# himhan34/Intensity_based_LiDAR_SLAM_for_me-

Measured on AMD Instinct MI355X. Metric: scans/sec (64×1024 Ouster) feature+kNN+residual path; pose Δ vs CPU ref, higher is better.
Workload: dtype fp32 features / fp64 residual+solve

## Files before the change

include/lislam.h:

```cpp
#ifndef LISLAM_H_
#define LISLAM_H_

#include <stddef.h>
#include <stdint.h>

#ifdef __cplusplus
extern "C" {
#endif

#define LISLAM_OK 0
#define LISLAM_ERR_ARG (-1)
#define LISLAM_ERR_DEVICE (-2)
#define LISLAM_ERR_CAPACITY (-3)
#define LISLAM_ERR_STATE (-4)

typedef struct lislam_ctx lislam_ctx;
typedef struct lislam_batch lislam_batch;
typedef struct lislam_odom lislam_odom;

typedef struct {
  int32_t n_scans;
  int32_t width;
  float min_range;
  int32_t max_iterations;
// ... 57 lines not shown
#define LISLAM_OUT_LASER_CLOUD 3
#define LISLAM_OUT_CURVATURE 4
#define LISLAM_OUT_LABEL 5
#define LISLAM_OUT_LINE_OFFSETS 6
#define LISLAM_OUT_SHARP 7
#define LISLAM_OUT_LESS_SHARP 8
#define LISLAM_OUT_FLAT 9
#define LISLAM_OUT_LESS_FLAT 10
#define LISLAM_OUT_PARA 11
#define LISLAM_OUT_POSE 12
#define LISLAM_OUT_STATS 13
#define LISLAM_OUT_ORB_T 14
#define LISLAM_OUT_ORB_STATS 15
#define LISLAM_OUT_ORB_KEYPOINTS 16
#define LISLAM_OUT_ORB_POINTS 17
#define LISLAM_OUT_ORB_DESCRIPTORS 18
#define LISLAM_OUT_GROUND 19
#define LISLAM_OUT_GROUND_PLANE 20
#define LISLAM_OUT_GROUND_INFO 21
int lislam_batch_download(lislam_batch* b, int32_t what, int32_t scan, void* dst, int32_t cap, int32_t* n);
int lislam_batch_download_cloud(lislam_batch* b, int32_t what, int32_t scan, void* dst, const lislam_point_layout* layout,
                                int32_t cap, int32_t* n);

#define LISLAM_ENGINE_OFF 0
#define LISLAM_ENGINE_AUTO 1
#define LISLAM_ENGINE_ON 2
int lislam_set_odometry_schedule(lislam_ctx* ctx, int32_t mode);
int lislam_set_engine_shape(lislam_ctx* ctx, int32_t queries_per_wave, int32_t depth);
#define LISLAM_PAIRING_OFF 0
#define LISLAM_PAIRING_AUTO 1
#define LISLAM_PAIRING_REQUIRE 2
int lislam_set_engine_pairing(lislam_ctx* ctx, int32_t mode);
int lislam_batch_odometry_paired(lislam_batch* b, int32_t* paired);
int lislam_batch_odometry_status(lislam_batch* b, int32_t* status);
int lislam_batch_odometry_engine(lislam_batch* b, int32_t* kind);
int lislam_batch_odometry_abort_code(lislam_batch* b, int32_t* code);
int lislam_device_queue_count(int32_t device, int32_t* masked_queues);

#define LISLAM_TIES_REFERENCE 0
#define LISLAM_TIES_INDEX 1
int lislam_set_tie_order(lislam_ctx* ctx, int32_t order);

int lislam_eval_factors(lislam_ctx* ctx, int32_t n, const int32_t* kind, const double* pts, const double* q,
                        const double* t, double* residuals, double* jac);
int lislam_eval_factors_raw(lislam_ctx* ctx, int32_t n, const int32_t* kind, const double* pts, const double* q,
                            const double* t, double* residuals, double* jac_q, double* jac_t);
// ... 145 lines not shown
```

intensity_based_lidar_slam_for_me-_amd/csrc/lislam_abi.cpp:

```cpp
#include <hip/hip_runtime.h>

#include <algorithm>
#include <atomic>
#include <cstdarg>
#include <cstdio>
#include <cstdlib>
#include <cstring>
#include <string>
#include <vector>

#include "../../include/lislam.h"
#include "lislam_batch.hpp"
#include "lislam_ctx.hpp"
#include "lislam_internal.hpp"

using namespace lislam;


namespace {

int fail(lislam_ctx* c, int code, const char* fmt, ...) {
  if (c) {
    char buf[512];
    va_list ap;
// ... 655 lines not shown
}

int lislam_batch_odometry_engine(lislam_batch* b, int32_t* kind) {
  if (!b || !kind) return LISLAM_ERR_ARG;
  *kind = !b->engine_ran ? 0 : b->eng_split == 1 ? 2 : 1;
  return LISLAM_OK;
}

int lislam_batch_kernel_times(lislam_batch* b, float* ms_per_call, int32_t* launches_per_call, int32_t* calls) {
  if (!b || !ms_per_call) return LISLAM_ERR_ARG;
  SETTLE(b);
  lislam_ctx* c = b->ctx;
  hipSetDevice(c->device);
  HIPCHK(c, hipStreamSynchronize(c->stream));
  double acc[LISLAM_NUM_KERNELS] = {0};
  int launches[LISLAM_NUM_KERNELS] = {0};
  auto el = [&](hipEvent_t a0, hipEvent_t a1) -> double {
    float ms = 0;
    if (hipEventElapsedTime(&ms, a0, a1) != hipSuccess) return 0.0;
    return ms;
  };
  for (auto& v : b->ext_ev) {
    timeline_print(c->device, "extract", b, 0, v[0], v[4]);
    for (int i = 0; i < 4; i++) { acc[i] += el(v[i], v[i + 1]); launches[i] += i == 3 ? 2 : i == 0 ? 3 : 1; }
    for (hipEvent_t e : v) b->pool.push_back(e);
  }
  for (auto& v : b->odo_ev) {
    for (auto& t : v) {
      timeline_print(c->device, "odometry", b, t.kernel, t.b, t.e);
      acc[t.kernel] += el(t.b, t.e);
      launches[t.kernel] += 1;
      b->pool.push_back(t.b);
      b->pool.push_back(t.e);
    }
  }
  const int ne = (int)b->ext_ev.size(), no = (int)b->odo_ev.size();
  for (int k = 0; k < LISLAM_NUM_KERNELS; k++) {
    const int ncall = k < 4 ? ne : no;
    ms_per_call[k] = ncall ? (float)(acc[k] / ncall) : 0.f;
    if (launches_per_call) launches_per_call[k] = ncall ? launches[k] / ncall : 0;
  }
  if (calls) { calls[0] = ne; calls[1] = no; }
  b->ext_ev.clear();
  b->odo_ev.clear();
  return LISLAM_OK;
}

// ... 151 lines not shown
  if (info && (rc = lislam_batch_download(b, LISLAM_OUT_GROUND_INFO, 0, info, 4, &n))) return rc;
  if (out) {
    if ((rc = lislam_batch_download(b, LISLAM_OUT_GROUND, 0, out, cap, &n))) return rc;
    if (n_out) *n_out = n;
  }
  return LISLAM_OK;
}

int lislam_odom_create(lislam_ctx* c, lislam_odom** out) {
  if (!c || !out) return LISLAM_ERR_ARG;
  hipSetDevice(c->device);
  int rc = ensure_single(c);
  if (rc) return rc;
  *out = new lislam_odom();
  (*out)->ctx = c;
  return LISLAM_OK;
}

int lislam_odom_destroy(lislam_odom* od) {
  delete od;
  return LISLAM_OK;
}

static int put_frame(lislam_batch* b, int slot, const lislam_frame* fr) {
  lislam_ctx* c = b->ctx;
  if (fr->n_sharp > b->cap_sharp || fr->n_less_sharp > b->cap_less_sharp || fr->n_flat > b->cap_flat ||
      fr->n_less_flat > b->N || fr->n_sharp < 0 || fr->n_less_sharp < 0 || fr->n_flat < 0 || fr->n_less_flat < 0)
    return fail(c, LISLAM_ERR_CAPACITY, "frame exceeds feature capacities");
  const FeatureArgs& f = b->fa;
  auto cp = [&](P4* dst, const float* src, int n) -> int {
    if (n > 0) HIPCHK(c, hipMemcpyAsync(dst, src, (size_t)n * 16, hipMemcpyHostToDevice, c->stream));
    return LISLAM_OK;
  };
  int rc = 0;
  rc |= cp(f.sharp + (size_t)slot * b->cap_sharp, fr->sharp, fr->n_sharp);
  rc |= cp(f.less_sharp + (size_t)slot * b->cap_less_sharp, fr->less_sharp, fr->n_less_sharp);
  rc |= cp(f.flat + (size_t)slot * b->cap_flat, fr->flat, fr->n_flat);
  rc |= cp(f.less_flat + (size_t)slot * b->N, fr->less_flat, fr->n_less_flat);
  const int cnt[4] = {fr->n_sharp, fr->n_less_sharp, fr->n_flat, fr->n_less_flat};
  HIPCHK(c, hipMemcpyAsync(f.n_feat + slot * 4, cnt, sizeof(cnt), hipMemcpyHostToDevice, c->stream));
  const int H = b->H;
  std::vector<int> loff(2 * (H + 1));
  const float* src[2] = {fr->less_sharp, fr->less_flat};
  const int nsrc[2] = {fr->n_less_sharp, fr->n_less_flat};
  for (int w = 0; w < 2; w++) {
    int j = 0;
    for (int l = 0; l <= H; l++) {
      while (j < nsrc[w] && (l == H || (int)src[w][4 * j + 3] < l)) j++;
      loff[w * (H + 1) + l] = j;
    }
  }
  HIPCHK(c, hipMemcpyAsync(f.feat_loff + (size_t)slot * 2 * (H + 1), loff.data(), loff.size() * sizeof(int),
                           hipMemcpyHostToDevice, c->stream));
  OdomArgs o = b->oa;
  o.less_sharp = f.less_sharp + (size_t)slot * b->cap_less_sharp;
  o.less_flat = f.less_flat + (size_t)slot * b->N;
  o.sharp = f.sharp + (size_t)slot * b->cap_sharp;
  o.flat = f.flat + (size_t)slot * b->cap_flat;
  o.qpts_sharp += (size_t)slot * b->cap_sharp;
  o.qpts_flat += (size_t)slot * b->cap_flat;
  o.n_feat = f.n_feat + slot * 4;
  for (TargetIndex* ti : {&o.idx_ls, &o.idx_lf}) {
    ti->chunk += (size_t)slot * ti->nchunk * 2;
    ti->super += (size_t)slot * ti->nsuper * 2;
    ti->nn_chunk += (size_t)slot * ti->nchunk * 2;
    ti->nn_super += (size_t)slot * ti->nsuper * 2;
    ti->sorted += (size_t)slot * ti->cap;
    ti->keys += (size_t)slot * 2 * ti->cap;
  }
  launch_target_index(o, 1, c->stream);
  HIPCHK(c, hipGetLastError());
  HIPCHK(c, hipStreamSynchronize(c->stream));
  return rc ? LISLAM_ERR_DEVICE : LISLAM_OK;
}

static int copy_slot(lislam_batch* b, int from, int to) {
  lislam_ctx* c = b->ctx;
  const hipStream_t st = c->stream;
  auto cp = [&](const void* base, size_t per_slot) -> int {
    const char* p = static_cast<const char*>(base);
    HIPCHK(c, hipMemcpyAsync(const_cast<char*>(p) + (size_t)to * per_slot, p + (size_t)from * per_slot, per_slot,
                             hipMemcpyDeviceToDevice, st));
    return LISLAM_OK;
  };
  const FeatureArgs& f = b->fa;
  const OdomArgs& o = b->oa;
  int rc = 0;
  rc |= cp(f.sharp, (size_t)b->cap_sharp * 16);
  rc |= cp(f.less_sharp, (size_t)b->cap_less_sharp * 16);
  rc |= cp(f.flat, (size_t)b->cap_flat * 16);
  rc |= cp(f.less_flat, (size_t)b->N * 16);
  rc |= cp(f.n_feat, 4 * sizeof(int));
  rc |= cp(f.feat_loff, (size_t)2 * (b->H + 1) * sizeof(int));
  for (const TargetIndex* ti : {&o.idx_ls, &o.idx_lf}) {
// ... 165 lines not shown
```

intensity_based_lidar_slam_for_me-_amd/csrc/lislam_internal.hpp:

```cpp
#pragma once
#include <hip/hip_runtime.h>
#include <stdint.h>

#include <atomic>
#include <chrono>
#include <vector>

#include "lislam_device.hpp"

namespace lislam {

constexpr int kMaxLines = 128;
constexpr int kCapSharpPerLine = 12;
constexpr int kCapLessSharpPerLine = 120;
constexpr int kCapFlatPerLine = 24;
constexpr int kMaxEngineDepth = 6;

struct FeatureArgs {
  const P4* pts;
  int S, H, W, N;
  float min_range;
  uint8_t* img_range;
  uint8_t* img_int;
  P4* track;
// ... 61 lines not shown
  const int* gate;
  unsigned* eng_ctl;
  int eng_qpw, eng_depth;
  int* warm;
  double* eng_part;
};

struct FactorArgs {
  int n;
  const int* kind;
  const double* pts;
  const double* x;
  double* res;
  double* jac;
};

struct WireLayout {
  uint32_t step, ox, oy, oz, oi;
};
void launch_unpack_layout(const uint8_t* raw, int n, const WireLayout& L, P4* out, hipStream_t st);
void launch_pack_layout(const P4* in, int n, const WireLayout& L, uint8_t* raw, hipStream_t st);

void launch_features(const FeatureArgs& a, hipStream_t st, hipEvent_t* ev , hipEvent_t images_ready);
void launch_target_index(const OdomArgs& a, int n_scans, hipStream_t st);
struct OdoTimed {
  int kernel;
  hipEvent_t b, e;
};
void launch_odometry(const OdomArgs& a, const hipStream_t* streams, int ngroups, hipEvent_t fork,
                     const hipEvent_t* join, std::vector<OdoTimed>* ev, hipEvent_t (*get_event)(void*),
                     void* ev_owner);
int launch_odometry_chain(const OdomArgs& a, hipStream_t st);
int launch_odometry_chain_split(const OdomArgs& a, hipEvent_t ready, hipEvent_t fork, hipEvent_t join_r,
                                hipEvent_t join_i, hipEvent_t t0, hipEvent_t t1, unsigned* h_abort, hipEvent_t done);
struct EngineRequest {
  OdomArgs a;
  hipEvent_t ready, fork, join_r, join_i, t0, t1, done;
  unsigned* h_abort;
  void* plan = nullptr;
  std::atomic<int> state{0};
  int pairing = 0;
  size_t ctl_words = 0;
  bool paired = false;
  bool held = false;
  std::chrono::steady_clock::time_point hold_t0;
};
// ... 28 lines not shown
```

intensity_based_lidar_slam_for_me-_amd/csrc/lislam_odometry.hip:

```cpp
#include <hip/hip_runtime.h>
#include <hip/hip_ext.h>

#include <algorithm>
#include <atomic>
#include <cassert>
#include <chrono>
#include <condition_variable>
#include <cstdlib>
#include <cstring>
#include <deque>
#include <mutex>
#include <thread>
#include <vector>

#include "lislam_device.hpp"
#include "lislam_factors.hpp"
#include "lislam_internal.hpp"
#include "lislam_lm.hpp"
#include "lislam_lm_wave.hpp"

namespace lislam {

__device__ __forceinline__ int uni(int v) { return __builtin_amdgcn_readfirstlane(v); }

constexpr double kDistSq = 25.0;
constexpr double kNearby = 2.5;


__device__ __forceinline__ uint32_t spread10(uint32_t v) {
  v &= 0x3ffu;
  v = (v | (v << 16)) & 0x030000FFu;
  v = (v | (v << 8)) & 0x0300F00Fu;
  v = (v | (v << 4)) & 0x030C30C3u;
  v = (v | (v << 2)) & 0x09249249u;
  return v;
}

__device__ __forceinline__ void stg4(float4* p, float4 v) {
  f4v w = {v.x, v.y, v.z, v.w};
  *(gf4v_mut*)p = w;
}

__device__ __forceinline__ void chunk_boxes(const float4* pts, int n, bool label_from_w, float4* chunk, float4* super) {
  const int nch = (n + kChunk - 1) / kChunk;
  for (int c = threadIdx.x; c < nch; c += blockDim.x) {
    float4 lo = make_float4(3.4e38f, 3.4e38f, 3.4e38f, 1e9f), hi = make_float4(-3.4e38f, -3.4e38f, -3.4e38f, -1e9f);
    for (int j = c * kChunk; j < min(n, c * kChunk + kChunk); j++) {
      const float4 p = ldg(pts + j);
      const float l = label_from_w ? (float)int(p.w) : 0.f;
      lo.x = fminf(lo.x, p.x); lo.y = fminf(lo.y, p.y); lo.z = fminf(lo.z, p.z); lo.w = fminf(lo.w, l);
      hi.x = fmaxf(hi.x, p.x); hi.y = fmaxf(hi.y, p.y); hi.z = fmaxf(hi.z, p.z); hi.w = fmaxf(hi.w, l);
    }
    stg4(chunk + 2 * c, lo);
    stg4(chunk + 2 * c + 1, hi);
  }
  __syncthreads();
  const int nsu = (nch + kChunk - 1) / kChunk;
  for (int c = threadIdx.x; c < nsu; c += blockDim.x) {
    float4 lo = make_float4(3.4e38f, 3.4e38f, 3.4e38f, 1e9f), hi = make_float4(-3.4e38f, -3.4e38f, -3.4e38f, -1e9f);
    for (int k = c * kChunk; k < min(nch, c * kChunk + kChunk); k++) {
      const float4 l = ldg(chunk + 2 * k), h = ldg(chunk + 2 * k + 1);
      lo.x = fminf(lo.x, l.x); lo.y = fminf(lo.y, l.y); lo.z = fminf(lo.z, l.z); lo.w = fminf(lo.w, l.w);
      hi.x = fmaxf(hi.x, h.x); hi.y = fmaxf(hi.y, h.y); hi.z = fmaxf(hi.z, h.z); hi.w = fmaxf(hi.w, h.w);
    }
    stg4(super + 2 * c, lo);
    stg4(super + 2 * c + 1, hi);
  }
  __syncthreads();
}

typedef __attribute__((address_space(1))) uint64_t gu64;

__device__ __forceinline__ void global_bitonic(gu64* keys, int P) {
  for (int k = 2; k <= P; k <<= 1) {
    for (int j = k >> 1; j > 0; j >>= 1) {
      for (int i = threadIdx.x; i < P; i += blockDim.x) {
        const int ixj = i ^ j;
        if (ixj > i) {
          const uint64_t x = keys[i], y = keys[ixj];
          if ((x > y) == ((i & k) == 0)) { keys[i] = y; keys[ixj] = x; }
        }
      }
      __syncthreads();
    }
  }
}

template <int kW, int kK>
__device__ __forceinline__ void wg_bitonic(uint64_t (&key)[kK], int P, uint64_t* xch) {
  constexpr int kPer = 64 * kK;
  const int w = threadIdx.x >> 6, lane = lane_id();
  const bool active = w * kPer < P;
  const int base = w * kPer;
  for (int k = 2; k <= P; k <<= 1) {
    for (int j = k >> 1; j >= kPer; j >>= 1) {
      const int pw = w ^ (j / kPer);
      const bool up = (base & k) == 0, lower = (w & (j / kPer)) == 0;
#pragma unroll
      for (int h = 0; h < kK / 8; h++) {
        if (active)
#pragma unroll
          for (int t = 0; t < 8; t++) xch[(w * 8 + t) * 64 + lane] = key[h * 8 + t];
        __syncthreads();
        if (active)
#pragma unroll
          for (int t = 0; t < 8; t++) {
            const uint64_t x = key[h * 8 + t], y = xch[(pw * 8 + t) * 64 + lane];
            key[h * 8 + t] = (lower == up) ? (x < y ? x : y) : (x < y ? y : x);
          }
        __syncthreads();
      }
    }
    if (active) reg_bitonic_level<kK>(key, k, min(k >> 1, kPer / 2), base);
  }
}

#ifndef LISLAM_TI_WPE32
#define LISLAM_TI_WPE32 4
#endif
template <int kW, int kK>
__device__ __forceinline__ void target_index_body(const OdomArgs& a, int bid, int per_scan, int w0, int w1, int w2,
                                                  uint64_t* xch, float (*red)[kW]) {
  constexpr int kKeysPerLane = kK, kPer = 64 * kK;
  const int s = bid / per_scan, wi = bid % per_scan;
  const int which = wi == 0 ? w0 : wi == 1 ? w1 : w2;
  const bool query = which >= 2;
  const TargetIndex& ix = (which & 1) ? a.idx_lf : a.idx_ls;
  const float4* pts = reinterpret_cast<const float4*>(
      which == 0 ? a.less_sharp + (size_t)s * a.cap_less_sharp : which == 1 ? a.less_flat + (size_t)s * a.N
      : which == 2 ? a.sharp + (size_t)s * a.cap_sharp : a.flat + (size_t)s * a.cap_flat);
  const int n = a.n_feat[s * 4 + (which == 0 ? 1 : which == 1 ? 3 : which == 2 ? 0 : 2)];
  if (!query) chunk_boxes(pts, n, true, ix.chunk + (size_t)s * ix.nchunk * 2, ix.super + (size_t)s * ix.nsuper * 2);
  if (n == 0) return;
  float mn[3] = {3.4e38f, 3.4e38f, 3.4e38f}, mx[3] = {-3.4e38f, -3.4e38f, -3.4e38f};
  if (!query) {
    const float4* sb = ix.super + (size_t)s * ix.nsuper * 2;
    const int nsu = ((n + kChunk - 1) / kChunk + kChunk - 1) / kChunk;
    for (int u = threadIdx.x; u < nsu; u += 64 * kW) {
      const float4 l = ldg(sb + 2 * u), h = ldg(sb + 2 * u + 1);
      mn[0] = fminf(mn[0], l.x); mn[1] = fminf(mn[1], l.y); mn[2] = fminf(mn[2], l.z);
      mx[0] = fmaxf(mx[0], h.x); mx[1] = fmaxf(mx[1], h.y); mx[2] = fmaxf(mx[2], h.z);
    }
  } else {
    for (int j = threadIdx.x; j < n; j += 64 * kW) {
      const float4 p = ldg(pts + j);
      mn[0] = fminf(mn[0], p.x); mn[1] = fminf(mn[1], p.y); mn[2] = fminf(mn[2], p.z);
      mx[0] = fmaxf(mx[0], p.x); mx[1] = fmaxf(mx[1], p.y); mx[2] = fmaxf(mx[2], p.z);
    }
  }
  for (int d = 0; d < 3; d++)
    for (int o = 32; o > 0; o >>= 1) {
      mn[d] = fminf(mn[d], __shfl_xor(mn[d], o));
      mx[d] = fmaxf(mx[d], __shfl_xor(mx[d], o));
    }
  const int lane = threadIdx.x & 63, wave = threadIdx.x >> 6;
// ... 35 lines not shown
      for (int t = 0; t < kKeysPerLane; t++) {
        const int i = wave * kPer + t * 64 + lane;
        if (i < n) f(i, (int)(uint32_t)key[t]);
      }
    } else {
      for (int i = threadIdx.x; i < n; i += 64 * kW) f(i, (int)(uint32_t)gkeys[i]);
    }
  };
  if (query) {
    float4* qp = which == 2 ? a.qpts_sharp + (size_t)s * a.cap_sharp : a.qpts_flat + (size_t)s * a.cap_flat;
    emit([&](int i, int o) {
      const float4 p = ldg(pts + o);
      stg4(qp + i, make_float4(p.x, p.y, p.z, __int_as_float(o)));
    });
    return;
  }
  float4* sorted = ix.sorted + (size_t)s * ix.cap;
  if (!in_regs) {
    emit([&](int i, int o) {
      const float4 p = ldg(pts + o);
      stg4(sorted + i, make_float4(p.x, p.y, p.z, __int_as_float(o)));
    });
    __syncthreads();
    chunk_boxes(sorted, n, false, ix.nn_chunk + (size_t)s * ix.nchunk * 2, ix.nn_super + (size_t)s * ix.nsuper * 2);
    return;
  }
  float4* nch_out = ix.nn_chunk + (size_t)s * ix.nchunk * 2;
  float4* nsu_out = ix.nn_super + (size_t)s * ix.nsuper * 2;
  auto rmin = [](float v) {
    v = fminf(v, __int_as_float(__builtin_amdgcn_mov_dpp(__float_as_int(v), 0xB1, 0xf, 0xf, true)));
    v = fminf(v, __int_as_float(__builtin_amdgcn_mov_dpp(__float_as_int(v), 0x4E, 0xf, 0xf, true)));
    v = fminf(v, __int_as_float(__builtin_amdgcn_mov_dpp(__float_as_int(v), 0x141, 0xf, 0xf, true)));
    return fminf(v, __int_as_float(__builtin_amdgcn_mov_dpp(__float_as_int(v), 0x140, 0xf, 0xf, true)));
  };
  float slo[3] = {3.4e38f, 3.4e38f, 3.4e38f}, shi[3] = {-3.4e38f, -3.4e38f, -3.4e38f};
#pragma unroll
  for (int t = 0; t < kKeysPerLane; t++) {
    const int i = wave * kPer + t * 64 + lane;
    float4 p = make_float4(3.4e38f, 3.4e38f, 3.4e38f, 0.f);
    float q[3] = {-3.4e38f, -3.4e38f, -3.4e38f};
    if (i < n) {
      const int o = (int)(uint32_t)key[t];
      p = ldg(pts + o);
      stg4(sorted + i, make_float4(p.x, p.y, p.z, __int_as_float(o)));
      q[0] = p.x; q[1] = p.y; q[2] = p.z;
    }
    const float lo0 = rmin(p.x), lo1 = rmin(p.y), lo2 = rmin(p.z);
    const float hi0 = -rmin(-q[0]), hi1 = -rmin(-q[1]), hi2 = -rmin(-q[2]);
    const int c = i >> 4;
    if ((lane & 15) == 0 && i < n) {
      stg4(nch_out + 2 * c, make_float4(lo0, lo1, lo2, 0.f));
      stg4(nch_out + 2 * c + 1, make_float4(hi0, hi1, hi2, 0.f));
    }
    slo[0] = fminf(slo[0], lo0); slo[1] = fminf(slo[1], lo1); slo[2] = fminf(slo[2], lo2);
    shi[0] = fmaxf(shi[0], hi0); shi[1] = fmaxf(shi[1], hi1); shi[2] = fmaxf(shi[2], hi2);
    if ((t & 3) == 3) {
      float r[6] = {slo[0], slo[1], slo[2], -shi[0], -shi[1], -shi[2]};
#pragma unroll
      for (int e = 0; e < 6; e++) {
        float v = r[e];
        v = fminf(v, __int_as_float(__builtin_amdgcn_ds_swizzle(__float_as_int(v), (16 << 10) | 0x1f)));
        v = fminf(v, __shfl_xor(v, 32));
        r[e] = v;
      }
      const int u = (wave * kPer + (t - 3) * 64) >> 8;
      if (lane == 0 && u * kSuper < n) {
        stg4(nsu_out + 2 * u, make_float4(r[0], r[1], r[2], 0.f));
        stg4(nsu_out + 2 * u + 1, make_float4(-r[3], -r[4], -r[5], 0.f));
      }
      slo[0] = slo[1] = slo[2] = 3.4e38f;
      shi[0] = shi[1] = shi[2] = -3.4e38f;
    }
  }
}

template <int kW, int kK>
__global__ __launch_bounds__(64 * kW, kK >= 32 ? LISLAM_TI_WPE32 : 4) void k_target_index(OdomArgs a, int per_scan, int w0, int w1, int w2) {
  __shared__ uint64_t xch[kW * 8 * 64];
  __shared__ float red[6][kW];
  target_index_body<kW, kK>(a, blockIdx.x, per_scan, w0, w1, w2, xch, red);
}

__global__ __launch_bounds__(512, LISLAM_TI_WPE32) void k_target_index_all(OdomArgs a, int n_scans) {
  __shared__ uint64_t xch[8 * 8 * 64];
  __shared__ float red[6][8];
  if ((int)blockIdx.x < n_scans)
    target_index_body<8, 32>(a, blockIdx.x, 1, 1, 1, 1, xch, red);
  else
    target_index_body<8, 16>(a, blockIdx.x - n_scans, 3, 0, 2, 3, xch, red);
}

__device__ __forceinline__ P4 transform_to_start(const P4& pi, const double* x) {
  const DQ q{x[0], x[1], x[2], x[3]};
  const D3 u = qrot(q, D3{(double)pi.x, (double)pi.y, (double)pi.z}) + D3{1.0 * x[4], 1.0 * x[5], 1.0 * x[6]};
  return P4{(float)u.x, (float)u.y, (float)u.z, pi.i};
}

__device__ __forceinline__ float d2f(const P4& q, const P4& p) {
  const float dx = q.x - p.x, dy = q.y - p.y, dz = q.z - p.z;
  return dx * dx + dy * dy + dz * dz;
}

__device__ __forceinline__ float box_lb(const float4& lo, const float4& hi, const P4& q) {
  const float dx = fmaxf(fmaxf(lo.x - q.x, q.x - hi.x), 0.f);
  const float dy = fmaxf(fmaxf(lo.y - q.y, q.y - hi.y), 0.f);
  const float dz = fmaxf(fmaxf(lo.z - q.z, q.z - hi.z), 0.f);
  return dx * dx + dy * dy + dz * dz;
}


#ifdef LISLAM_PHASE_PROF
__device__ unsigned long long g_assoc_stats[16];
// ... 2866 lines not shown
  r->state.store(1);
  g->q.push_back(r);
  g->cv_req.notify_one();
  return 1;
}

void wait_engine_launched(EngineRequest* r) {
  if (r->state.load() != 1) return;
  int dev = 0;
  (void)hipGetDevice(&dev);
  EngineGate* g = engine_gate(dev);
  std::unique_lock<std::mutex> lk(g->mu);
  g->cv_launched.wait(lk, [&] { return r->state.load() != 1; });
}

void launch_factors_raw(const RawFactorArgs& a, hipStream_t st) {
  if (a.n > 0) hipLaunchKernelGGL(k_eval_factors_raw, dim3((a.n + 255) / 256), dim3(256), 0, st, a);
}

void launch_factors(const FactorArgs& a, hipStream_t st) {
  if (a.n > 0) hipLaunchKernelGGL(k_eval_factors, dim3((a.n + 255) / 256), dim3(256), 0, st, a);
}

void launch_target_index(const OdomArgs& a, int n_scans, hipStream_t st) {
  static const bool split = getenv("LISLAM_TI_SPLIT") && atoi(getenv("LISLAM_TI_SPLIT")) == 1;
  if (!split) {
    hipLaunchKernelGGL(k_target_index_all, dim3(4 * n_scans), dim3(512), 0, st, a, n_scans);
    return;
  }
  hipLaunchKernelGGL((k_target_index<8, 32>), dim3(n_scans), dim3(512), 0, st, a, 1, 1, 1, 1);
  hipLaunchKernelGGL((k_target_index<8, 16>), dim3(3 * n_scans), dim3(512), 0, st, a, 3, 0, 2, 3);
}

void launch_odometry(const OdomArgs& a0, const hipStream_t* streams, int ngroups, hipEvent_t fork,
                     const hipEvent_t* join, std::vector<OdoTimed>* ev, hipEvent_t (*get_event)(void*),
                     void* owner) {
  if (a0.n_chains <= 0) return;
  const hipStream_t st = streams[0];
  hipLaunchKernelGGL(k_odom_init, dim3((a0.n_chains + 63) / 64), dim3(64), 0, st, a0);
  const int G = max(1, min(ngroups, a0.n_chains));
  if (G > 1) {
    (void)hipEventRecord(fork, st);
    for (int g = 1; g < G; g++) (void)hipStreamWaitEvent(streams[g], fork, 0);
  }
  const int qblocks16 = (a0.cap_sharp + a0.cap_flat + 8 - 1) / 8;
  const int rounds = min(a0.chain_len, a0.S - 1);
  auto timed = [&](int kernel, hipStream_t s, auto&& launch) {
    hipEvent_t b = nullptr, e = nullptr;
    if (ev) { b = get_event(owner); (void)hipEventRecord(b, s); }
    launch();
    if (ev) { e = get_event(owner); (void)hipEventRecord(e, s); ev->push_back({kernel, b, e}); }
  };
  for (int r = 0; r < rounds; r++) {
    for (int outer = 0; outer < 2; outer++) {
// ... 25 lines not shown
```

intensity_based_lidar_slam_for_me-_amd/frontend.py:

```python
from __future__ import annotations

import ctypes
from dataclasses import dataclass

import numpy as np

from . import native as nat

CAP_SHARP_PER_LINE, CAP_LESS_SHARP_PER_LINE, CAP_FLAT_PER_LINE = 12, 120, 24

PACKED_XYZI = nat.PointLayout(16, 0, 4, 8, 12)
OUSTER_LAYOUT = nat.PointLayout(48, 0, 4, 8, 16)
PCL_XYZI_LAYOUT = nat.PointLayout(32, 0, 4, 8, 16)


class Context:

    def __init__(self, n_scans: int = 64, width: int = 1024, min_range: float = 0.3, max_iterations: int = 4,
                 want_images: bool = True, device: int = 0):
        self.lib = nat.load()
        self.n_scans, self.width, self.device = n_scans, width, device
        cfg = nat.Config(n_scans, width, min_range, max_iterations, int(want_images))
        h = ctypes.c_void_p()
        rc = self.lib.lislam_ctx_create(ctypes.byref(cfg), device, ctypes.byref(h))
# ... 253 lines not shown
        cap = max(N, 16)
        buf = np.zeros((cap, w) if w > 1 else cap, dt)
        n = ctypes.c_int32()
        rc = self.ctx.lib.lislam_batch_download(self.h, what, scan, nat.ptr(buf), cap, ctypes.byref(n))
        nat.check(rc, self.ctx.h, "lislam_batch_download")
        return buf[: n.value].copy()

    def count(self, what: int, scan: int) -> int:
        n = ctypes.c_int32()
        nat.check(self.ctx.lib.lislam_batch_download(self.h, what, scan, None, 0, ctypes.byref(n)), self.ctx.h,
                  "lislam_batch_download")
        return n.value

    def download_cloud(self, what: int, scan: int, layout: nat.PointLayout | None = None) -> bytes:
        lay = layout or PCL_XYZI_LAYOUT
        cap = max(self.ctx.n_scans * self.ctx.width, 16)
        buf = np.zeros(cap * lay.point_step, np.uint8)
        n = ctypes.c_int32()
        rc = self.ctx.lib.lislam_batch_download_cloud(self.h, what, scan, nat.ptr(buf), ctypes.byref(lay), cap,
                                                      ctypes.byref(n))
        nat.check(rc, self.ctx.h, "lislam_batch_download_cloud")
        return buf[: n.value * lay.point_step].tobytes()

    def features(self, scan: int) -> Features:
        return Features(self.download(nat.OUT_LASER_CLOUD, scan), self.download(nat.OUT_SHARP, scan),
                        self.download(nat.OUT_LESS_SHARP, scan), self.download(nat.OUT_FLAT, scan),
                        self.download(nat.OUT_LESS_FLAT, scan))

    def close(self):
        if self.h:
            self.ctx.lib.lislam_batch_destroy(self.h)
            self.h = None


def eval_factors(ctx: Context, kind: np.ndarray, pts: np.ndarray, q: np.ndarray, t: np.ndarray):
    kind = np.ascontiguousarray(kind, np.int32)
    pts = np.ascontiguousarray(pts, np.float64).reshape(-1, 12)
    n = kind.shape[0]
    r = np.zeros((n, 3))
    J = np.zeros((n, 3, 6))
    rc = ctx.lib.lislam_eval_factors(ctx.h, n, nat.ptr(kind), nat.ptr(pts), nat.ptr(np.ascontiguousarray(q, np.float64)),
                                     nat.ptr(np.ascontiguousarray(t, np.float64)), nat.ptr(r), nat.ptr(J))
    nat.check(rc, ctx.h, "lislam_eval_factors")
    return r, J
```

intensity_based_lidar_slam_for_me-_amd/native.py:

```python
from __future__ import annotations

import ctypes
import os

import numpy as np

HERE = os.path.dirname(os.path.abspath(__file__))
LIB_PATH = os.path.join(HERE, "liblislam.so")

OK = 0
ERR_ARG, ERR_DEVICE, ERR_CAPACITY, ERR_STATE = -1, -2, -3, -4

OUT_IMAGE_RANGE, OUT_IMAGE_INTENSITY, OUT_CLOUD_TRACK, OUT_LASER_CLOUD = 0, 1, 2, 3
OUT_CURVATURE, OUT_LABEL, OUT_LINE_OFFSETS = 4, 5, 6
OUT_SHARP, OUT_LESS_SHARP, OUT_FLAT, OUT_LESS_FLAT = 7, 8, 9, 10
OUT_PARA, OUT_POSE, OUT_STATS = 11, 12, 13
OUT_ORB_T, OUT_ORB_STATS, OUT_ORB_KEYPOINTS, OUT_ORB_POINTS, OUT_ORB_DESCRIPTORS = 14, 15, 16, 17, 18
OUT_GROUND, OUT_GROUND_PLANE, OUT_GROUND_INFO = 19, 20, 21

KERNELS = ("k_scan_front", "k_scan_lines", "k_scan_compact", "k_target_index", "k_odom_assoc", "k_odom_lm",
           "k_odom_chain")

EXPORTED_SYMBOLS = (
    "lislam_ctx_create", "lislam_ctx_destroy", "lislam_last_error", "lislam_synchronize",
    "lislam_set_stream", "lislam_get_stream", "lislam_scan_registration", "lislam_odom_create",
    "lislam_odom_destroy", "lislam_odom_step", "lislam_batch_create", "lislam_batch_destroy",
    "lislam_batch_upload", "lislam_batch_upload_async", "lislam_batch_download_cloud", "lislam_batch_input_device_ptr", "lislam_batch_extract",
    "lislam_batch_odometry", "lislam_batch_set_timing", "lislam_batch_kernel_times",
    "lislam_batch_download", "lislam_eval_factors", "lislam_eval_factors_raw", "lislam_set_tie_order", "lislam_set_odometry_schedule", "lislam_set_engine_shape", "lislam_batch_odometry_status",
    "lislam_batch_odometry_engine", "lislam_batch_odometry_abort_code", "lislam_device_queue_count",
    "lislam_set_engine_pairing", "lislam_batch_odometry_paired",
    "lislam_map_create", "lislam_map_destroy", "lislam_map_build", "lislam_map_add_points", "lislam_map_size",
    "lislam_map_points", "lislam_map_nearest_search", "lislam_map_associate", "lislam_normal_equations",
    "lislam_pose_solve", "lislam_voxel_grid", "lislam_mapopt_step", "lislam_mapopt_step_corner", "lislam_laser_mapping",
    "lislam_map_set_timing", "lislam_map_kernel_times",
    "lislam_orb_detect", "lislam_orb_match", "lislam_intensity_tracker_create", "lislam_intensity_tracker_destroy",
    "lislam_intensity_tracker_step", "lislam_batch_intensity_odometry", "lislam_batch_orb_cascade_info", "lislam_batch_ground", "lislam_ground_extract",
    "lislam_lmap_create", "lislam_lmap_destroy", "lislam_lmap_step", "lislam_lmap_counts", "lislam_lmap_points",
    "lislam_batch_odometry_gated", "lislam_odom_step_gated", "lislam_batch_mapopt", "lislam_batch_mapopt_corner", "lislam_loop_icp", "lislam_odom_fuser_create", "lislam_odom_fuser_destroy", "lislam_odom_fuse",
    "lislam_place_create", "lislam_place_destroy", "lislam_place_size", "lislam_place_add_clouds", "lislam_place_add_batch",
    "lislam_place_detect", "lislam_place_distance", "lislam_place_download",
    "lislam_pgo_create", "lislam_pgo_destroy", "lislam_pgo_size", "lislam_pgo_add_nodes", "lislam_pgo_set_prior",
    "lislam_pgo_add_edges", "lislam_pgo_add_batch", "lislam_pgo_edges", "lislam_pgo_linearize", "lislam_pgo_optimize",
    "lislam_pgo_poses",
)

MAP_KERNELS = ("k_knn", "k_fit", "k_lm_eval", "k_lm_step", "map_rebuild", "map_downsample", "k_orb_pyramid",
               "k_orb_fast", "k_orb_select", "k_orb_finish", "k_orb_blur", "k_orb_desc", "k_orb_match", "k_orb_lm",
               "k_ground_screen", "k_ground_ransac", "k_ground_extract", "k_lc_step", "k_lc_apply", "k_fuse",
               "k_orb_roiblur", "k_lm_solve")

MATCH_LINE, MATCH_PLANE = 0, 1
PLACE_DESC, PLACE_RING_KEY, PLACE_SECTOR_KEY = 0, 1, 2
PLACE_KERNELS = ("k_sc_describe", "k_sc_finish", "k_sc_detect", "k_sc_distance")
# ... 105 lines not shown
    L.lislam_odom_step.argtypes = [vp, ctypes.POINTER(Frame), vp, vp, vp]
    L.lislam_batch_create.argtypes = [vp, _i32, ctypes.POINTER(vp)]
    L.lislam_batch_destroy.argtypes = [vp]
    L.lislam_batch_upload.argtypes = [vp, vp, _i32, ctypes.POINTER(PointLayout)]
    L.lislam_batch_upload_async.argtypes = [vp, vp, _i32, ctypes.POINTER(PointLayout)]
    L.lislam_batch_input_device_ptr.argtypes = [vp, ctypes.POINTER(vp)]
    L.lislam_batch_extract.argtypes = [vp, _i32]
    L.lislam_batch_odometry.argtypes = [vp, _i32, _i32]
    L.lislam_batch_set_timing.argtypes = [vp, _i32]
    L.lislam_batch_kernel_times.argtypes = [vp, _fp, _i32p, _i32p]
    L.lislam_batch_download.argtypes = [vp, _i32, _i32, vp, _i32, _i32p]
    L.lislam_batch_download_cloud.argtypes = [vp, _i32, _i32, vp, ctypes.POINTER(PointLayout), _i32, _i32p]
    L.lislam_eval_factors.argtypes = [vp, _i32, vp, vp, vp, vp, vp, vp]
    L.lislam_eval_factors_raw.argtypes = [vp, _i32, vp, vp, vp, vp, vp, vp, vp]
    L.lislam_set_tie_order.argtypes = [vp, _i32]
    L.lislam_set_odometry_schedule.argtypes = [vp, _i32]
    L.lislam_set_engine_shape.argtypes = [vp, _i32, _i32]
    L.lislam_batch_odometry_status.argtypes = [vp, ctypes.POINTER(_i32)]
    L.lislam_batch_odometry_engine.argtypes = [vp, ctypes.POINTER(_i32)]
    L.lislam_set_engine_pairing.argtypes = [vp, _i32]
    L.lislam_batch_odometry_paired.argtypes = [vp, ctypes.POINTER(_i32)]
    L.lislam_batch_odometry_abort_code.argtypes = [vp, ctypes.POINTER(_i32)]
    L.lislam_device_queue_count.argtypes = [_i32, ctypes.POINTER(_i32)]
    i64, i64p = ctypes.c_int64, ctypes.POINTER(ctypes.c_int64)
    L.lislam_map_create.argtypes = [vp, ctypes.POINTER(MapConfig), ctypes.POINTER(vp)]
    L.lislam_map_destroy.argtypes = [vp]
    L.lislam_map_build.argtypes = [vp, vp, i64, _i32]
    L.lislam_map_add_points.argtypes = [vp, vp, i64, _i32, _i32, i64p]
    L.lislam_map_size.argtypes = [vp, i64p]
    L.lislam_map_points.argtypes = [vp, vp, i64, i64p]
    L.lislam_map_nearest_search.argtypes = [vp, vp, _i32, _i32, _i32, ctypes.c_float, vp, vp, vp]
    L.lislam_map_associate.argtypes = [vp, _i32, vp, _i32, _i32, vp, vp, vp]
    L.lislam_normal_equations.argtypes = [vp, vp, vp, _i32, vp, vp]
    L.lislam_pose_solve.argtypes = [vp, vp, vp, _i32, vp, _i32, vp]
    L.lislam_voxel_grid.argtypes = [vp, vp, _i32, ctypes.c_float, vp, _i32p]
    L.lislam_mapopt_step.argtypes = [vp, vp, _i32, vp, vp, vp, vp]
    L.lislam_mapopt_step_corner.argtypes = [vp, vp, vp, _i32, vp, _i32, vp, vp, vp, vp]
    L.lislam_laser_mapping.argtypes = [vp, vp, vp, _i32, vp, _i32, vp, vp]
    L.lislam_orb_detect.argtypes = [vp, vp, vp, vp, _i32, _i32, _i32, vp, vp, vp, _i32, _i32p]
    L.lislam_orb_match.argtypes = [vp, vp, _i32, vp, _i32, vp, _i32p]
    L.lislam_intensity_tracker_create.argtypes = [vp, _i32, _i32, _i32, vp, ctypes.POINTER(vp)]
    L.lislam_intensity_tracker_destroy.argtypes = [vp]
    L.lislam_intensity_tracker_step.argtypes = [vp, vp, vp, vp, vp]
    L.lislam_batch_intensity_odometry.argtypes = [vp, _i32, _i32, vp]
    L.lislam_batch_orb_cascade_info.argtypes = [vp, _i32p]
    L.lislam_batch_ground.argtypes = [vp, _i32]
# ... 58 lines not shown
```

Baseline: 30150.

## Size target-index kernels per feature kind and parallelize chunk box reduction

Replaces the single fused target-index kernel, which ran every feature kind at 512 threads and 32 keys per lane, with three launches whose block size and keys per lane are picked from each kind's capacity. Query and non-query paths become compile-time specializations. Chunk and super-chunk bounding boxes are now built with a 16-lane DPP min reduction across lanes instead of a serial loop per thread. The aim is to stop small sets (sharp, flat, less-sharp) from paying for an 8-wave sort and to raise occupancy, at the cost of two extra kernel launches per call. A debug entry point for inspecting the index is also added.

New measurement: 30050. No clear change (-0.3%).

```diff
diff --git a/include/lislam.h b/include/lislam.h
--- a/include/lislam.h
+++ b/include/lislam.h
@@ -103,6 +103,9 @@
 int lislam_batch_download_cloud(lislam_batch* b, int32_t what, int32_t scan, void* dst, const lislam_point_layout* layout,
                                 int32_t cap, int32_t* n);
 
+int lislam_debug_target_index(lislam_batch* b, int32_t scan, int32_t which, const float* cloud, int32_t n_cloud,
+                              float* sorted, float* chunk, float* super, float* nn_chunk, float* nn_super, int32_t* n);
+
 #define LISLAM_ENGINE_OFF 0
 #define LISLAM_ENGINE_AUTO 1
 #define LISLAM_ENGINE_ON 2
diff --git a/intensity_based_lidar_slam_for_me-_amd/csrc/lislam_abi.cpp b/intensity_based_lidar_slam_for_me-_amd/csrc/lislam_abi.cpp
--- a/intensity_based_lidar_slam_for_me-_amd/csrc/lislam_abi.cpp
+++ b/intensity_based_lidar_slam_for_me-_amd/csrc/lislam_abi.cpp
@@ -701,7 +701,7 @@
   };
   for (auto& v : b->ext_ev) {
     timeline_print(c->device, "extract", b, 0, v[0], v[4]);
-    for (int i = 0; i < 4; i++) { acc[i] += el(v[i], v[i + 1]); launches[i] += i == 3 ? 2 : i == 0 ? 3 : 1; }
+    for (int i = 0; i < 4; i++) { acc[i] += el(v[i], v[i + 1]); launches[i] += i == 3 ? lislam::kTargetIndexLaunches : i == 0 ? 3 : 1; }
     for (hipEvent_t e : v) b->pool.push_back(e);
   }
   for (auto& v : b->odo_ev) {
@@ -899,6 +899,27 @@
   return LISLAM_OK;
 }
 
+static OdomArgs slot_index_args(const lislam_batch* b, int slot) {
+  const FeatureArgs& f = b->fa;
+  OdomArgs o = b->oa;
+  o.less_sharp = f.less_sharp + (size_t)slot * b->cap_less_sharp;
+  o.less_flat = f.less_flat + (size_t)slot * b->N;
+  o.sharp = f.sharp + (size_t)slot * b->cap_sharp;
+  o.flat = f.flat + (size_t)slot * b->cap_flat;
+  o.qpts_sharp += (size_t)slot * b->cap_sharp;
+  o.qpts_flat += (size_t)slot * b->cap_flat;
+  o.n_feat = f.n_feat + slot * 4;
+  for (TargetIndex* ti : {&o.idx_ls, &o.idx_lf}) {
+    ti->chunk += (size_t)slot * ti->nchunk * 2;
+    ti->super += (size_t)slot * ti->nsuper * 2;
+    ti->nn_chunk += (size_t)slot * ti->nchunk * 2;
+    ti->nn_super += (size_t)slot * ti->nsuper * 2;
+    ti->sorted += (size_t)slot * ti->cap;
+    ti->keys += (size_t)slot * 2 * ti->cap;
+  }
+  return o;
+}
+
 static int put_frame(lislam_batch* b, int slot, const lislam_frame* fr) {
   lislam_ctx* c = b->ctx;
   if (fr->n_sharp > b->cap_sharp || fr->n_less_sharp > b->cap_less_sharp || fr->n_flat > b->cap_flat ||
@@ -929,24 +950,52 @@
   }
   HIPCHK(c, hipMemcpyAsync(f.feat_loff + (size_t)slot * 2 * (H + 1), loff.data(), loff.size() * sizeof(int),
                            hipMemcpyHostToDevice, c->stream));
-  OdomArgs o = b->oa;
-  o.less_sharp = f.less_sharp + (size_t)slot * b->cap_less_sharp;
-  o.less_flat = f.less_flat + (size_t)slot * b->N;
-  o.sharp = f.sharp + (size_t)slot * b->cap_sharp;
-  o.flat = f.flat + (size_t)slot * b->cap_flat;
-  o.qpts_sharp += (size_t)slot * b->cap_sharp;
-  o.qpts_flat += (size_t)slot * b->cap_flat;
-  o.n_feat = f.n_feat + slot * 4;
-  for (TargetIndex* ti : {&o.idx_ls, &o.idx_lf}) {
-    ti->chunk += (size_t)slot * ti->nchunk * 2;
-    ti->super += (size_t)slot * ti->nsuper * 2;
-    ti->nn_chunk += (size_t)slot * ti->nchunk * 2;
-    ti->nn_super += (size_t)slot * ti->nsuper * 2;
-    ti->sorted += (size_t)slot * ti->cap;
-    ti->keys += (size_t)slot * 2 * ti->cap;
-  }
-  launch_target_index(o, 1, c->stream);
+  launch_target_index(slot_index_args(b, slot), 1, c->stream);
   HIPCHK(c, hipGetLastError());
+  HIPCHK(c, hipStreamSynchronize(c->stream));
+  return rc ? LISLAM_ERR_DEVICE : LISLAM_OK;
+}
+
+int lislam_debug_target_index(lislam_batch* b, int32_t scan, int32_t which, const float* cloud, int32_t n_cloud,
+                              float* sorted, float* chunk, float* super, float* nn_chunk, float* nn_super, int32_t* n) {
+  if (!b || scan < 0 || scan >= b->extracted || which < 0 || which > 3 || !n) return LISLAM_ERR_ARG;
+  SETTLE(b);
+  lislam_ctx* c = b->ctx;
+  hipSetDevice(c->device);
+  const FeatureArgs& f = b->fa;
+  const OdomArgs& o = b->oa;
+  const int cap = which == 0 ? b->cap_less_sharp : which == 1 ? b->N : which == 2 ? b->cap_sharp : b->cap_flat;
+  const int cnt_at = scan * 4 + (which == 0 ? 1 : which == 1 ? 3 : which == 2 ? 0 : 2);
+  if (cloud) {
+    if (n_cloud < 0 || n_cloud > cap) return fail(c, LISLAM_ERR_CAPACITY, "cloud exceeds the kind's capacity");
+    P4* dst = which == 0 ? f.less_sharp : which == 1 ? f.less_flat : which == 2 ? f.sharp : f.flat;
+    if (n_cloud > 0)
+      HIPCHK(c, hipMemcpyAsync(dst + (size_t)scan * cap, cloud, (size_t)n_cloud * 16, hipMemcpyHostToDevice, c->stream));
+    HIPCHK(c, hipMemcpyAsync(f.n_feat + cnt_at, &n_cloud, sizeof(int), hipMemcpyHostToDevice, c->stream));
+    HIPCHK(c, hipStreamSynchronize(c->stream));
+    launch_target_index(slot_index_args(b, scan), 1, c->stream);
+    HIPCHK(c, hipGetLastError());
+  }
+  int cnt = 0;
+  HIPCHK(c, hipMemcpyAsync(&cnt, f.n_feat + cnt_at, sizeof(int), hipMemcpyDeviceToHost, c->stream));
+  HIPCHK(c, hipStreamSynchronize(c->stream));
+  *n = cnt;
+  auto get = [&](float* dst, const float4* src, size_t count) -> int {
+    if (dst && count) HIPCHK(c, hipMemcpyAsync(dst, src, count * 16, hipMemcpyDeviceToHost, c->stream));
+    return LISLAM_OK;
+  };
+  int rc = 0;
+  if (which >= 2) {
+    rc |= get(sorted, (which == 2 ? o.qpts_sharp : o.qpts_flat) + (size_t)scan * cap, cnt);
+  } else {
+    const TargetIndex& ti = which == 1 ? o.idx_lf : o.idx_ls;
+    const size_t nch = (cnt + lislam::kChunk - 1) / lislam::kChunk, nsu = (nch + lislam::kChunk - 1) / lislam::kChunk;
+    rc |= get(sorted, ti.sorted + (size_t)scan * ti.cap, cnt);
+    rc |= get(chunk, ti.chunk + (size_t)scan * ti.nchunk * 2, nch * 2);
+    rc |= get(super, ti.super + (size_t)scan * ti.nsuper * 2, nsu * 2);
+    rc |= get(nn_chunk, ti.nn_chunk + (size_t)scan * ti.nchunk * 2, nch * 2);
+    rc |= get(nn_super, ti.nn_super + (size_t)scan * ti.nsuper * 2, nsu * 2);
+  }
   HIPCHK(c, hipStreamSynchronize(c->stream));
   return rc ? LISLAM_ERR_DEVICE : LISLAM_OK;
 }
diff --git a/intensity_based_lidar_slam_for_me-_amd/csrc/lislam_internal.hpp b/intensity_based_lidar_slam_for_me-_amd/csrc/lislam_internal.hpp
--- a/intensity_based_lidar_slam_for_me-_amd/csrc/lislam_internal.hpp
+++ b/intensity_based_lidar_slam_for_me-_amd/csrc/lislam_internal.hpp
@@ -107,6 +107,7 @@
 void launch_pack_layout(const P4* in, int n, const WireLayout& L, uint8_t* raw, hipStream_t st);
 
 void launch_features(const FeatureArgs& a, hipStream_t st, hipEvent_t* ev , hipEvent_t images_ready);
+constexpr int kTargetIndexLaunches = 3;
 void launch_target_index(const OdomArgs& a, int n_scans, hipStream_t st);
 struct OdoTimed {
   int kernel;
diff --git a/intensity_based_lidar_slam_for_me-_amd/csrc/lislam_odometry.hip b/intensity_based_lidar_slam_for_me-_amd/csrc/lislam_odometry.hip
--- a/intensity_based_lidar_slam_for_me-_amd/csrc/lislam_odometry.hip
+++ b/intensity_based_lidar_slam_for_me-_amd/csrc/lislam_odometry.hip
@@ -41,30 +41,46 @@
   *(gf4v_mut*)p = w;
 }
 
+__device__ __forceinline__ float row_min16(float v) {
+  v = fminf(v, __int_as_float(__builtin_amdgcn_mov_dpp(__float_as_int(v), 0xB1, 0xf, 0xf, true)));
+  v = fminf(v, __int_as_float(__builtin_amdgcn_mov_dpp(__float_as_int(v), 0x4E, 0xf, 0xf, true)));
+  v = fminf(v, __int_as_float(__builtin_amdgcn_mov_dpp(__float_as_int(v), 0x141, 0xf, 0xf, true)));
+  return fminf(v, __int_as_float(__builtin_amdgcn_mov_dpp(__float_as_int(v), 0x140, 0xf, 0xf, true)));
+}
+
+template <int kT>
 __device__ __forceinline__ void chunk_boxes(const float4* pts, int n, bool label_from_w, float4* chunk, float4* super) {
   const int nch = (n + kChunk - 1) / kChunk;
-  for (int c = threadIdx.x; c < nch; c += blockDim.x) {
-    float4 lo = make_float4(3.4e38f, 3.4e38f, 3.4e38f, 1e9f), hi = make_float4(-3.4e38f, -3.4e38f, -3.4e38f, -1e9f);
-    for (int j = c * kChunk; j < min(n, c * kChunk + kChunk); j++) {
+  for (int j = threadIdx.x; j < nch * kChunk; j += kT) {
+    float lo[4] = {3.4e38f, 3.4e38f, 3.4e38f, 1e9f}, nhi[4] = {3.4e38f, 3.4e38f, 3.4e38f, 1e9f};
+    if (j < n) {
       const float4 p = ldg(pts + j);
       const float l = label_from_w ? (float)int(p.w) : 0.f;
-      lo.x = fminf(lo.x, p.x); lo.y = fminf(lo.y, p.y); lo.z = fminf(lo.z, p.z); lo.w = fminf(lo.w, l);
-      hi.x = fmaxf(hi.x, p.x); hi.y = fmaxf(hi.y, p.y); hi.z = fmaxf(hi.z, p.z); hi.w = fmaxf(hi.w, l);
-    }
-    stg4(chunk + 2 * c, lo);
-    stg4(chunk + 2 * c + 1, hi);
+      lo[0] = p.x; lo[1] = p.y; lo[2] = p.z; lo[3] = l;
+      nhi[0] = -p.x; nhi[1] = -p.y; nhi[2] = -p.z; nhi[3] = -l;
+    }
+#pragma unroll
+    for (int e = 0; e < 4; e++) { lo[e] = row_min16(lo[e]); nhi[e] = row_min16(nhi[e]); }
+    if ((j & (kChunk - 1)) == 0) {
+      stg4(chunk + 2 * (j >> 4), make_float4(lo[0], lo[1], lo[2], lo[3]));
+      stg4(chunk + 2 * (j >> 4) + 1, make_float4(-nhi[0], -nhi[1], -nhi[2], -nhi[3]));
+    }
   }
   __syncthreads();
   const int nsu = (nch + kChunk - 1) / kChunk;
-  for (int c = threadIdx.x; c < nsu; c += blockDim.x) {
-    float4 lo = make_float4(3.4e38f, 3.4e38f, 3.4e38f, 1e9f), hi = make_float4(-3.4e38f, -3.4e38f, -3.4e38f, -1e9f);
-    for (int k = c * kChunk; k < min(nch, c * kChunk + kChunk); k++) {
+  for (int k = threadIdx.x; k < nsu * kChunk; k += kT) {
+    float lo[4] = {3.4e38f, 3.4e38f, 3.4e38f, 1e9f}, nhi[4] = {3.4e38f, 3.4e38f, 3.4e38f, 1e9f};
+    if (k < nch) {
       const float4 l = ldg(chunk + 2 * k), h = ldg(chunk + 2 * k + 1);
-      lo.x = fminf(lo.x, l.x); lo.y = fminf(lo.y, l.y); lo.z = fminf(lo.z, l.z); lo.w = fminf(lo.w, l.w);
-      hi.x = fmaxf(hi.x, h.x); hi.y = fmaxf(hi.y, h.y); hi.z = fmaxf(hi.z, h.z); hi.w = fmaxf(hi.w, h.w);
-    }
-    stg4(super + 2 * c, lo);
-    stg4(super + 2 * c + 1, hi);
+      lo[0] = l.x; lo[1] = l.y; lo[2] = l.z; lo[3] = l.w;
+      nhi[0] = -h.x; nhi[1] = -h.y; nhi[2] = -h.z; nhi[3] = -h.w;
+    }
+#pragma unroll
+    for (int e = 0; e < 4; e++) { lo[e] = row_min16(lo[e]); nhi[e] = row_min16(nhi[e]); }
+    if ((k & (kChunk - 1)) == 0) {
+      stg4(super + 2 * (k >> 4), make_float4(lo[0], lo[1], lo[2], lo[3]));
+      stg4(super + 2 * (k >> 4) + 1, make_float4(-nhi[0], -nhi[1], -nhi[2], -nhi[3]));
+    }
   }
   __syncthreads();
 }
@@ -93,7 +109,7 @@
   const bool active = w * kPer < P;
   const int base = w * kPer;
   for (int k = 2; k <= P; k <<= 1) {
-    for (int j = k >> 1; j >= kPer; j >>= 1) {
+    for (int j = k >> 1; kW > 1 && j >= kPer; j >>= 1) {
       const int pw = w ^ (j / kPer);
       const bool up = (base & k) == 0, lower = (w & (j / kPer)) == 0;
 #pragma unroll
@@ -118,19 +134,20 @@
 #ifndef LISLAM_TI_WPE32
 #define LISLAM_TI_WPE32 4
 #endif
-template <int kW, int kK>
-__device__ __forceinline__ void target_index_body(const OdomArgs& a, int bid, int per_scan, int w0, int w1, int w2,
-                                                  uint64_t* xch, float (*red)[kW]) {
+#ifndef LISLAM_TI_WPE16
+#define LISLAM_TI_WPE16 6
+#endif
+template <int kW, int kK, bool kQuery>
+__device__ __forceinline__ void target_index_body(const OdomArgs& a, int s, int which, uint64_t* xch, float (*red)[kW]) {
   constexpr int kKeysPerLane = kK, kPer = 64 * kK;
-  const int s = bid / per_scan, wi = bid % per_scan;
-  const int which = wi == 0 ? w0 : wi == 1 ? w1 : w2;
-  const bool query = which >= 2;
+  constexpr bool query = kQuery;
   const TargetIndex& ix = (which & 1) ? a.idx_lf : a.idx_ls;
   const float4* pts = reinterpret_cast<const float4*>(
       which == 0 ? a.less_sharp + (size_t)s * a.cap_less_sharp : which == 1 ? a.less_flat + (size_t)s * a.N
       : which == 2 ? a.sharp + (size_t)s * a.cap_sharp : a.flat + (size_t)s * a.cap_flat);
   const int n = a.n_feat[s * 4 + (which == 0 ? 1 : which == 1 ? 3 : which == 2 ? 0 : 2)];
-  if (!query) chunk_boxes(pts, n, true, ix.chunk + (size_t)s * ix.nchunk * 2, ix.super + (size_t)s * ix.nsuper * 2);
+  if (!query)
+    chunk_boxes<64 * kW>(pts, n, true, ix.chunk + (size_t)s * ix.nchunk * 2, ix.super + (size_t)s * ix.nsuper * 2);
   if (n == 0) return;
   float mn[3] = {3.4e38f, 3.4e38f, 3.4e38f}, mx[3] = {-3.4e38f, -3.4e38f, -3.4e38f};
   if (!query) {
@@ -212,17 +229,12 @@
       stg4(sorted + i, make_float4(p.x, p.y, p.z, __int_as_float(o)));
     });
     __syncthreads();
-    chunk_boxes(sorted, n, false, ix.nn_chunk + (size_t)s * ix.nchunk * 2, ix.nn_super + (size_t)s * ix.nsuper * 2);
+    chunk_boxes<64 * kW>(sorted, n, false, ix.nn_chunk + (size_t)s * ix.nchunk * 2, ix.nn_super + (size_t)s * ix.nsuper * 2);
     return;
   }
   float4* nch_out = ix.nn_chunk + (size_t)s * ix.nchunk * 2;
   float4* nsu_out = ix.nn_super + (size_t)s * ix.nsuper * 2;
-  auto rmin = [](float v) {
-    v = fminf(v, __int_as_float(__builtin_amdgcn_mov_dpp(__float_as_int(v), 0xB1, 0xf, 0xf, true)));
-    v = fminf(v, __int_as_float(__builtin_amdgcn_mov_dpp(__float_as_int(v), 0x4E, 0xf, 0xf, true)));
-    v = fminf(v, __int_as_float(__builtin_amdgcn_mov_dpp(__float_as_int(v), 0x141, 0xf, 0xf, true)));
-    return fminf(v, __int_as_float(__builtin_amdgcn_mov_dpp(__float_as_int(v), 0x140, 0xf, 0xf, true)));
-  };
+  auto rmin = [](float v) { return row_min16(v); };
   float slo[3] = {3.4e38f, 3.4e38f, 3.4e38f}, shi[3] = {-3.4e38f, -3.4e38f, -3.4e38f};
 #pragma unroll
   for (int t = 0; t < kKeysPerLane; t++) {
@@ -264,20 +276,12 @@
   }
 }
 
-template <int kW, int kK>
-__global__ __launch_bounds__(64 * kW, kK >= 32 ? LISLAM_TI_WPE32 : 4) void k_target_index(OdomArgs a, int per_scan, int w0, int w1, int w2) {
-  __shared__ uint64_t xch[kW * 8 * 64];
+template <int kW, int kK, bool kQuery>
+__global__ __launch_bounds__(64 * kW, kK >= 32 ? LISLAM_TI_WPE32 : LISLAM_TI_WPE16) void k_target_index(OdomArgs a, int per_scan, int w0, int w1) {
+  __shared__ uint64_t xch[kW > 1 ? kW * 8 * 64 : 1];
   __shared__ float red[6][kW];
-  target_index_body<kW, kK>(a, blockIdx.x, per_scan, w0, w1, w2, xch, red);
-}
-
-__global__ __launch_bounds__(512, LISLAM_TI_WPE32) void k_target_index_all(OdomArgs a, int n_scans) {
-  __shared__ uint64_t xch[8 * 8 * 64];
-  __shared__ float red[6][8];
-  if ((int)blockIdx.x < n_scans)
-    target_index_body<8, 32>(a, blockIdx.x, 1, 1, 1, 1, xch, red);
-  else
-    target_index_body<8, 16>(a, blockIdx.x - n_scans, 3, 0, 2, 3, xch, red);
+  const int s = (int)blockIdx.x / per_scan;
+  target_index_body<kW, kK, kQuery>(a, s, (int)blockIdx.x - s * per_scan ? w1 : w0, xch, red);
 }
 
 __device__ __forceinline__ P4 transform_to_start(const P4& pi, const double* x) {
@@ -3190,14 +3194,34 @@
   if (a.n > 0) hipLaunchKernelGGL(k_eval_factors, dim3((a.n + 255) / 256), dim3(256), 0, st, a);
 }
 
+#ifndef LISLAM_TI_8K_WAVES
+#define LISLAM_TI_8K_WAVES 8
+#endif
+static int ti_shape(int cap) {
+  int shape = 0;
+  for (int P = 1024; P < cap && shape < 4; P <<= 1) shape++;
+  return shape;
+}
+
+template <bool kQuery>
+static void launch_ti_kinds(int shape, const OdomArgs& a, int per_scan, int w0, int w1, int n_scans, hipStream_t st) {
+  const dim3 grid(per_scan * n_scans);
+  switch (shape) {
+    case 0: hipLaunchKernelGGL((k_target_index<1, 16, kQuery>), grid, dim3(64), 0, st, a, per_scan, w0, w1); break;
+    case 1: hipLaunchKernelGGL((k_target_index<2, 16, kQuery>), grid, dim3(128), 0, st, a, per_scan, w0, w1); break;
+    case 2: hipLaunchKernelGGL((k_target_index<4, 16, kQuery>), grid, dim3(256), 0, st, a, per_scan, w0, w1); break;
+    case 3:
+      hipLaunchKernelGGL((k_target_index<LISLAM_TI_8K_WAVES, 128 / LISLAM_TI_8K_WAVES, kQuery>), grid,
+                         dim3(64 * LISLAM_TI_8K_WAVES), 0, st, a, per_scan, w0, w1);
+      break;
+    default: hipLaunchKernelGGL((k_target_index<8, 32, kQuery>), grid, dim3(512), 0, st, a, per_scan, w0, w1); break;
+  }
+}
+
 void launch_target_index(const OdomArgs& a, int n_scans, hipStream_t st) {
-  static const bool split = getenv("LISLAM_TI_SPLIT") && atoi(getenv("LISLAM_TI_SPLIT")) == 1;
-  if (!split) {
-    hipLaunchKernelGGL(k_target_index_all, dim3(4 * n_scans), dim3(512), 0, st, a, n_scans);
-    return;
-  }
-  hipLaunchKernelGGL((k_target_index<8, 32>), dim3(n_scans), dim3(512), 0, st, a, 1, 1, 1, 1);
-  hipLaunchKernelGGL((k_target_index<8, 16>), dim3(3 * n_scans), dim3(512), 0, st, a, 3, 0, 2, 3);
+  launch_ti_kinds<false>(ti_shape(a.N), a, 1, 1, 1, n_scans, st);
+  launch_ti_kinds<false>(ti_shape(a.cap_less_sharp), a, 1, 0, 0, n_scans, st);
+  launch_ti_kinds<true>(ti_shape(max(a.cap_flat, a.cap_sharp)), a, 2, 3, 2, n_scans, st);
 }
 
 void launch_odometry(const OdomArgs& a0, const hipStream_t* streams, int ngroups, hipEvent_t fork,
diff --git a/intensity_based_lidar_slam_for_me-_amd/frontend.py b/intensity_based_lidar_slam_for_me-_amd/frontend.py
--- a/intensity_based_lidar_slam_for_me-_amd/frontend.py
+++ b/intensity_based_lidar_slam_for_me-_amd/frontend.py
@@ -299,6 +299,29 @@
         nat.check(rc, self.ctx.h, "lislam_batch_download_cloud")
         return buf[: n.value * lay.point_step].tobytes()
 
+    def debug_target_index(self, scan: int, which: int, cloud: np.ndarray | None = None) -> dict:
+        H, N = self.ctx.n_scans, self.ctx.n_scans * self.ctx.width
+        cap = (20 * 6 * H, N, 2 * 6 * H, 4 * 6 * H)[which]
+        nch = (cap + 15) // 16
+        nsu = (nch + 15) // 16
+        out = {"sorted": np.zeros((max(cap, 1), 4), np.float32)}
+        if which < 2:
+            for name, m in (("chunk", nch), ("super", nsu), ("nn_chunk", nch), ("nn_super", nsu)):
+                out[name] = np.zeros((max(m, 1), 2, 4), np.float32)
+        c = None if cloud is None else np.ascontiguousarray(cloud, np.float32).reshape(-1, 4)
+        n = ctypes.c_int32()
+        rc = self.ctx.lib.lislam_debug_target_index(
+            self.h, scan, which, None if c is None else nat.ptr(c if c.shape[0] else np.zeros((1, 4), np.float32)),
+            0 if c is None else c.shape[0],
+            nat.ptr(out["sorted"]), *(nat.ptr(out[k]) if k in out else None for k in ("chunk", "super", "nn_chunk", "nn_super")),
+            ctypes.byref(n))
+        nat.check(rc, self.ctx.h, "lislam_debug_target_index")
+        n = n.value
+        mch = (n + 15) // 16
+        msu = (mch + 15) // 16
+        cut = {"sorted": n, "chunk": mch, "super": msu, "nn_chunk": mch, "nn_super": msu}
+        return {"n": n, **{k: v[: cut[k]].copy() for k, v in out.items()}}
+
     def features(self, scan: int) -> Features:
         return Features(self.download(nat.OUT_LASER_CLOUD, scan), self.download(nat.OUT_SHARP, scan),
                         self.download(nat.OUT_LESS_SHARP, scan), self.download(nat.OUT_FLAT, scan),
diff --git a/intensity_based_lidar_slam_for_me-_amd/native.py b/intensity_based_lidar_slam_for_me-_amd/native.py
--- a/intensity_based_lidar_slam_for_me-_amd/native.py
+++ b/intensity_based_lidar_slam_for_me-_amd/native.py
@@ -29,7 +29,7 @@
     "lislam_batch_odometry", "lislam_batch_set_timing", "lislam_batch_kernel_times",
     "lislam_batch_download", "lislam_eval_factors", "lislam_eval_factors_raw", "lislam_set_tie_order", "lislam_set_odometry_schedule", "lislam_set_engine_shape", "lislam_batch_odometry_status",
     "lislam_batch_odometry_engine", "lislam_batch_odometry_abort_code", "lislam_device_queue_count",
-    "lislam_set_engine_pairing", "lislam_batch_odometry_paired",
+    "lislam_set_engine_pairing", "lislam_batch_odometry_paired", "lislam_debug_target_index",
     "lislam_map_create", "lislam_map_destroy", "lislam_map_build", "lislam_map_add_points", "lislam_map_size",
     "lislam_map_points", "lislam_map_nearest_search", "lislam_map_associate", "lislam_normal_equations",
     "lislam_pose_solve", "lislam_voxel_grid", "lislam_mapopt_step", "lislam_mapopt_step_corner", "lislam_laser_mapping",
@@ -181,6 +181,7 @@
     L.lislam_batch_odometry_paired.argtypes = [vp, ctypes.POINTER(_i32)]
     L.lislam_batch_odometry_abort_code.argtypes = [vp, ctypes.POINTER(_i32)]
     L.lislam_device_queue_count.argtypes = [_i32, ctypes.POINTER(_i32)]
+    L.lislam_debug_target_index.argtypes = [vp, _i32, _i32, vp, _i32, vp, vp, vp, vp, vp, _i32p]
     i64, i64p = ctypes.c_int64, ctypes.POINTER(ctypes.c_int64)
     L.lislam_map_create.argtypes = [vp, ctypes.POINTER(MapConfig), ctypes.POINTER(vp)]
     L.lislam_map_destroy.argtypes = [vp]
```
